# MMintLab/gelslim_depth

Measured on AMD Instinct MI355X. Metric: train frames/sec (320x427) at batch 32, higher is better.
Workload: dtype f32

## Files before the change

### gelslim_depth_amd/csrc/gsd_conv3x3_w2d.hip

```cpp
#include "gsd_common.h"

#include <cstdio>
#include <cstdlib>
#include <type_traits>

__device__ const float gsd_pad_w2d[2] = {0.f, __builtin_nanf("")};

typedef float f32x4v __attribute__((ext_vector_type(4), aligned(4)));
typedef float f32x2v __attribute__((ext_vector_type(2)));

struct W2DParams {
  SrcD src0, src1;
  DstD dst0, dst1;
  const float* wt;
  float* partials;
  const float* bw_raw;
  const float* bw_scale;
  const float* bw_shift;
  const float* bw_mean;
  const float* bw_invstd;
  int Cin, Cout, Mpad, nchunks, mblocks;
  int N, H, W;
  int TH, TW, TWq, tiles_y, tiles_x, WR, WC, WCp, PS, NPV;
  int NP, NI;
  int mgrp, pgrp, ptiles;
  int nslab;
  float* slabs;
};

namespace {
constexpr int W2D_BM = 64;
constexpr int W2D_WTILE = 96 * W2D_BM;
constexpr int NWP = 2;
}

template <class GetY>
__device__ __forceinline__ void w2d_epilogue(const W2DParams& P, const float* sBw, const int n, const int h0, const int w0, const int tr2,
                                             const int tq, const int vmask, const int m0, const int mh, const int ph, const int j,
                                             const int l16, const int pt, GetY get_y) {
  constexpr int BM = 64;
  int off0_0 = 0, off0_1 = 0, off1_0 = 0, off1_1 = 0, sm0_0 = 0, sm0_1 = 0, sm1_0 = 0, sm1_1 = 0;
#pragma unroll
  for (int a = 0; a < 2; ++a) {
    const int h = h0 + 2 * tr2 + a, w = w0 + 4 * tq;
    const int vm = (vmask >> (4 * a)) & 15;
    int hd = h - P.dst0.oh, wd = w - P.dst0.ow;
    if ((unsigned)hd < (unsigned)P.dst0.H) {
      (a == 0 ? off0_0 : off0_1) = hd * P.dst0.ws + wd;
#pragma unroll
      for (int i = 0; i < 4; ++i)
        if ((vm >> i & 1) && (unsigned)(wd + i) < (unsigned)P.dst0.W) (a == 0 ? sm0_0 : sm0_1) |= 1 << i;
    }
    hd = h - P.dst1.oh;
    wd = w - P.dst1.ow;
    if ((unsigned)hd < (unsigned)P.dst1.H) {
      (a == 0 ? off1_0 : off1_1) = hd * P.dst1.ws + wd;
#pragma unroll
      for (int i = 0; i < 4; ++i)
        if ((vm >> i & 1) && (unsigned)(wd + i) < (unsigned)P.dst1.W) (a == 0 ? sm1_0 : sm1_1) |= 1 << i;
    }
  }
  auto OFF0 = [&](int a) { return a == 0 ? off0_0 : off0_1; };
  auto OFF1 = [&](int a) { return a == 0 ? off1_0 : off1_1; };
  auto SM0 = [&](int a) { return a == 0 ? sm0_0 : sm0_1; };
  auto SM1 = [&](int a) { return a == 0 ? sm1_0 : sm1_1; };
  const long long lane0 = (long long)(j * 4) * P.dst0.cs, lane1 = (long long)(j * 4) * P.dst1.cs;
  float* const d0 = P.dst0.p + (long long)n * P.dst0.ns;
  float* const d1 = P.dst1.p + (long long)n * P.dst1.ns;
  float* const prow = P.partials != nullptr ? P.partials + (size_t)(pt * NWP + ph) * (2 * P.Mpad) : nullptr;

  if (P.bw_raw == nullptr) {
#pragma unroll
    for (int m = 0; m < 2; ++m) {
#pragma unroll
      for (int reg = 0; reg < 4; ++reg) {
        const int cu = m0 + mh * 32 + m * 16 + reg, co = cu + j * 4;
        const bool first = co < P.dst0.C;
        const int cd = first ? co : co - P.dst0.C;
        const bool co_ok = co < P.Cout && (first || cd < P.dst1.C);
        float* const plane = first ? d0 + (long long)cu * P.dst0.cs + lane0 : d1 + (long long)(cu - P.dst0.C) * P.dst1.cs + lane1;
        float y[2][4];
        get_y(m, reg, y);
        float s1 = 0.f, s2 = 0.f;
#pragma unroll
        for (int a = 0; a < 2; ++a) {
          const int sm = co_ok ? (first ? SM0(a) : SM1(a)) : 0;
          float* const px = plane + (first ? OFF0(a) : OFF1(a));
#pragma unroll
          for (int i = 0; i < 4; ++i) {
            if (sm >> i & 1) {
              s1 += y[a][i];
              s2 = fmaf(y[a][i], y[a][i], s2);
            }
          }
          if (sm == 15) {
            *reinterpret_cast<f32x4v*>(px) = f32x4{y[a][0], y[a][1], y[a][2], y[a][3]};
          } else {
#pragma unroll
            for (int i = 0; i < 4; ++i)
              if (sm >> i & 1) px[i] = y[a][i];
          }
        }
        if (prow != nullptr) {
          s1 = reduce16_to_lane15(s1);
          s2 = reduce16_to_lane15(s2);
          if (l16 == 15 && co < P.Mpad) {
            prow[co] = s1;
            prow[P.Mpad + co] = s2;
          }
        }
      }
    }
  } else {
#pragma unroll
    for (int m = 0; m < 2; ++m) {
#pragma unroll
      for (int reg = 0; reg < 4; ++reg) {
        const int cu = m0 + mh * 32 + m * 16 + reg, co = cu + j * 4;
        const long long cplane = (long long)n * P.dst0.ns + (co < P.Cout ? (long long)cu * P.dst0.cs + lane0 : 0);
        float xr[2][4];
#pragma unroll
        for (int a = 0; a < 2; ++a) {
          const float* const rp = P.bw_raw + cplane + OFF0(a);
// ... 7 lines not shown
        }
        const int cl = mh * 32 + m * 16 + j * 4 + reg;
        const float bsc = sBw[cl], bsh = sBw[BM + cl], bmu = sBw[2 * BM + cl], bis = sBw[3 * BM + cl];
        float y[2][4];
        get_y(m, reg, y);
        float s1 = 0.f, s2 = 0.f;
#pragma unroll
        for (int a = 0; a < 2; ++a) {
          const int sm = co < P.Cout ? SM0(a) : 0;
          float* const px = d0 + ((long long)cu * P.dst0.cs + lane0) + OFF0(a);
#pragma unroll
          for (int i = 0; i < 4; ++i) {
            const float x = xr[a][i];
            const float dz = ((sm >> i & 1) && fmaf(x, bsc, bsh) > 0.f) ? y[a][i] : 0.f;
            y[a][i] = dz;
            s1 += dz;
            s2 = fmaf(dz, (x - bmu) * bis, s2);
          }
          if (sm == 15) {
            *reinterpret_cast<f32x4v*>(px) = f32x4{y[a][0], y[a][1], y[a][2], y[a][3]};
          } else {
#pragma unroll
            for (int i = 0; i < 4; ++i)
              if (sm >> i & 1) px[i] = y[a][i];
          }
        }
        if (prow != nullptr) {
          s1 = reduce16_to_lane15(s1);
          s2 = reduce16_to_lane15(s2);
          if (l16 == 15 && co < P.Mpad) {
            prow[co] = s1;
            prow[P.Mpad + co] = s2;
          }
        }
      }
    }
  }
}

template <bool PLAIN, int HM = 0, bool SPLIT = false>
__global__ __launch_bounds__(128 * NWP, 2) void conv3x3_w2d_kernel(const W2DParams P) {
  constexpr bool X4 = HM == 1, U4 = HM == 2, PC = HM != 0;
  constexpr int W2D_NONE = -2147483647 - 1, W2D_PAD = -2147483647;
  static_assert(!X4 || PLAIN, "aligned 16-byte halo pieces: a plain, row-pitched source");
  constexpr int BM = W2D_BM, WTILE = W2D_WTILE, NT = 128 * NWP, NW = 2 * NWP;
  extern __shared__ __attribute__((aligned(16))) float smem[];
  const int PS = P.PS;
  const int BUF = WTILE + 4 * PS;

  const int tid = threadIdx.x, lane = tid & 63;
  const int wave8 = __builtin_amdgcn_readfirstlane(tid >> 6);
  const int ph = wave8 % NWP, fh = wave8 / NWP;
  const int j = lane >> 4, l16 = lane & 15;

  const int lid = xcd_swizzle(blockIdx.x, gridDim.x);
  int mbb = lid % P.mblocks;
  const int slab = SPLIT ? (lid / P.mblocks) % P.nslab : 0;
  int pt = SPLIT ? lid / P.mblocks / P.nslab : lid / P.mblocks;
  if (!SPLIT && P.mgrp < P.mblocks) {
    const int gsz = P.pgrp * P.mblocks;
    const int g = lid / gsz;
    int r = lid - g * gsz;
    const int p0 = g * P.pgrp;
    const int pn = min(P.pgrp, P.ptiles - p0);
    const int per = pn * P.mgrp;
    const int mg = r / per;
    r -= mg * per;
    const int gn = min(P.mgrp, P.mblocks - mg * P.mgrp);
    const int pl = r / gn;
    pt = p0 + pl;
    mbb = mg * P.mgrp + (r - pl * gn);
  }
  const int c_lo = SPLIT ? (int)((long)slab * P.nchunks / P.nslab) : 0;
  const int c_hi = SPLIT ? (int)((long)(slab + 1) * P.nchunks / P.nslab) : P.nchunks;
  const int m0 = mbb * BM;
  const int tpi = P.tiles_y * P.tiles_x;
  const int n = pt / tpi;
  const int rt = pt - n * tpi;
  const int ty = rt / P.tiles_x;
  const int h0 = ty * P.TH, w0 = (rt - ty * P.tiles_x) * P.TW;

  const int q = ph * 16 + l16;
  const bool q_ok = q < (P.TH >> 1) * P.TWq && q < 16 * NWP;
  const int tr2 = q_ok ? q / P.TWq : 0;
  const int tq = q_ok ? q - tr2 * P.TWq : 0;
  const int baddr = WTILE + j * PS + (2 * tr2) * P.WCp + 4 * tq + (PC ? 4 : 0);
  int vmask = 0;
  if (q_ok) {
#pragma unroll
    for (int a = 0; a < 2; ++a)
      if (h0 + 2 * tr2 + a < P.H) {
#pragma unroll
        for (int i = 0; i < 4; ++i)
          if (w0 + 4 * tq + i < P.W) vmask |= 1 << (4 * a + i);
      }
  }

  bool p_on[2];
  int pmask = 0;
  auto seg_offsets = [&](const int seg, int (&xo)[2], const bool mark) __attribute__((always_inline)) {
    const SrcD& S = seg ? P.src1 : P.src0;
#pragma unroll
    for (int pp = 0; pp < 2; ++pp) {
      xo[pp] = W2D_NONE;
      if constexpr (PC) {
        const int u = wave8 + NW * pp;
        p_on[pp] = u < 4 * P.NI;
        const int piece = (u % P.NI) * 64 + lane;
        const int rr = piece / P.NP, pc = piece - rr * P.NP;
        if (rr < P.WR) {
          const int gh = h0 - 1 + rr, gw = w0 - 4 + 4 * pc;
          if constexpr (X4) {
            xo[pp] = ((unsigned)gh < (unsigned)S.H && gw >= 0 && gw + 4 <= S.ws) ? gh * S.ws + gw : W2D_PAD;
          } else {
            const int hs = gh - S.oh, c0 = gw - S.ow;
            xo[pp] = W2D_PAD;
            if (S.C > 0 && (unsigned)hs < (unsigned)S.H && c0 + 3 >= 0 && c0 < S.W) {
              xo[pp] = hs * S.ws + c0;
#pragma unroll
              for (int e = 0; e < 4; ++e)
                if (mark && (c0 + e < 0 || c0 + e >= S.W)) pmask |= 1 << (8 * seg + 4 * pp + e);
            }
          }
        }
        continue;
      }
      p_on[pp] = wave8 + NW * pp < P.NPV;
      const int pos = (wave8 + NW * pp) * 64 + lane;
      const int rr = pos / P.WCp, cc = pos - rr * P.WCp;
      if (rr < P.WR && cc < P.WC) {
        const int gh = h0 - 1 + rr, gw = w0 - 1 + cc;
        const int hs = gh - S.oh, ws = gw - S.ow;
        xo[pp] = ((unsigned)hs < (unsigned)S.H && (unsigned)ws < (unsigned)S.W) ? hs * S.ws + ws : W2D_PAD;
      }
    }
  };
  int xo0[2], xo1[2];
  seg_offsets(0, xo0, true);
  seg_offsets(1, xo1, true);
  const int f_sw = P.src1.C > 0 ? P.src0.C / 4 : -1;
  const bool start1 = SPLIT && f_sw >= 0 && c_lo >= f_sw;
  {
    const float pad0 = (start1 ? P.src1.relu : P.src0.relu) ? __builtin_nanf("") : 0.f;
#pragma unroll
    for (int pp = 0; pp < 2; ++pp)
      if (p_on[pp] && (start1 ? xo1[pp] : xo0[pp]) == W2D_PAD) {
#pragma unroll
        for (int b = 0; b < 2; ++b) {
          if constexpr (PC) {
            const int u = wave8 + NW * pp;
#pragma unroll
            for (int e = 0; e < 4; ++e) smem[b * BUF + WTILE + (u / P.NI) * PS + 1 + (u % P.NI) * 256 + lane * 4 + e] = pad0;
          } else {
#pragma unroll
            for (int ch = 0; ch < 4; ++ch) smem[b * BUF + WTILE + ch * PS + (wave8 + NW * pp) * 64 + lane] = pad0;
          }
        }
      }
  }
  long long d_cs = start1 ? P.src1.cs : P.src0.cs;
  const float* d_base = (start1 ? P.src1.p + (long long)n * P.src1.ns : P.src0.p + (long long)n * P.src0.ns) +
                        (long long)(c_lo - (start1 ? f_sw : 0)) * 4 * d_cs;
  long long f_xl[2];
#pragma unroll
  for (int pp = 0; pp < 2; ++pp) f_xl[pp] = start1 ? xo1[pp] : xo0[pp];
  auto begin_fill = [&](int chunk, int buf) {
    if (f_sw < 0 || start1 || (chunk != f_sw && chunk != f_sw + 1)) return;
// ... 221 lines not shown
  };
  for (int chunk = c_lo; chunk < c_hi; chunk += 2) {
    run_chunk(chunk, std::integral_constant<int, 0>{});
    if (chunk + 1 < c_hi) run_chunk(chunk + 1, std::integral_constant<int, 1>{});
  }

  {
    float* const xs = smem + (wave8 * 12) * 256 + lane * 4;
    const float* const xr = smem + ((ph + NWP * (1 - fh)) * 12) * 256 + lane * 4;
#pragma unroll
    for (int r = 0; r < 2; ++r) {
      __syncthreads();
#pragma unroll
      for (int f = 0; f < 12; ++f) *reinterpret_cast<f32x4*>(xs + f * 256) = acc[2 + r][f];
      __syncthreads();
#pragma unroll
      for (int f = 0; f < 12; ++f) acc[2 + r][f] = *reinterpret_cast<const f32x4*>(xr + f * 256);
    }
  }

  auto out_transform = [&](auto hi_c, int m, int reg, float (&y)[2][4]) __attribute__((always_inline)) {
    constexpr bool HI = decltype(hi_c)::value;
    const int lo = HI ? 2 + m : m, hi = HI ? m : 2 + m;
    const int r0 = reg & ~1;
#pragma unroll
    for (int a = 0; a < 2; ++a) {
      f32x2v R[6];
#pragma unroll
      for (int fc = 0; fc < 6; ++fc) {
        const f32x2v M0 = {acc[lo][fc][r0], acc[lo][fc][r0 + 1]}, M1 = {acc[lo][6 + fc][r0], acc[lo][6 + fc][r0 + 1]};
        const f32x2v M2 = {acc[hi][fc][r0], acc[hi][fc][r0 + 1]}, M3 = {acc[hi][6 + fc][r0], acc[hi][6 + fc][r0 + 1]};
        R[fc] = a == 0 ? M0 + M1 + M2 : M1 - M2 - M3;
      }
      const f32x2v p12 = R[1] + R[2], m12 = R[1] - R[2], p34 = R[3] + R[4], m34 = R[3] - R[4];
      const f32x2v c2 = {2.f, 2.f}, c4 = {4.f, 4.f}, c8 = {8.f, 8.f};
      const f32x2v y0 = R[0] + p12 + p34, y1 = __builtin_elementwise_fma(c2, m34, m12), y2 = __builtin_elementwise_fma(c4, p34, p12);
      const f32x2v y3 = __builtin_elementwise_fma(c8, m34, m12) + R[5];
      y[a][0] = y0[reg & 1], y[a][1] = y1[reg & 1], y[a][2] = y2[reg & 1], y[a][3] = y3[reg & 1];
    }
  };

  auto finish = [&](auto hi_c) __attribute__((always_inline)) {
    auto get_y = [&](int m, int reg, float (&y)[2][4]) __attribute__((always_inline)) { out_transform(hi_c, m, reg, y); };
    if constexpr (SPLIT) {
      float* const sl = P.slabs + ((size_t)((size_t)pt * P.nslab + slab) * P.mblocks + mbb) * (size_t)(BM * 128 * NWP);
#pragma unroll
      for (int m = 0; m < 2; ++m)
#pragma unroll
        for (int reg = 0; reg < 4; ++reg) {
          float y[2][4];
          get_y(m, reg, y);
          float* const o = sl + ((size_t)(fh * 32 + m * 16 + j * 4 + reg) * (16 * NWP) + q) * 8;
          *reinterpret_cast<f32x4*>(o) = f32x4{y[0][0], y[0][1], y[0][2], y[0][3]};
          *reinterpret_cast<f32x4*>(o + 4) = f32x4{y[1][0], y[1][1], y[1][2], y[1][3]};
        }
    } else {
      w2d_epilogue(P, sBw, n, h0, w0, tr2, tq, vmask, m0, fh, ph, j, l16, pt, get_y);
    }
  };
  if (fh == 0)
    finish(std::false_type{});
  else
    finish(std::true_type{});
}

__global__ __launch_bounds__(128 * NWP) void w2d_slab_reduce_kernel(const W2DParams P) {
  constexpr int BM = W2D_BM;
  __shared__ float sBw[4 * BM];
  const int tid = threadIdx.x, lane = tid & 63;
  const int wave8 = __builtin_amdgcn_readfirstlane(tid >> 6);
  const int ph = wave8 % NWP, mh = wave8 / NWP;
  const int j = lane >> 4, l16 = lane & 15;
  const int lid = xcd_swizzle(blockIdx.x, gridDim.x);
  const int mbb = lid % P.mblocks;
  const int pt = lid / P.mblocks;
  const int m0 = mbb * BM;
  const int tpi = P.tiles_y * P.tiles_x;
  const int n = pt / tpi;
  const int rt = pt - n * tpi;
  const int ty = rt / P.tiles_x;
  const int h0 = ty * P.TH, w0 = (rt - ty * P.tiles_x) * P.TW;
  const int q = ph * 16 + l16;
  const bool q_ok = q < (P.TH >> 1) * P.TWq && q < 16 * NWP;
  const int tr2 = q_ok ? q / P.TWq : 0;
  const int tq = q_ok ? q - tr2 * P.TWq : 0;
  int vmask = 0;
  if (q_ok) {
#pragma unroll
    for (int a = 0; a < 2; ++a)
      if (h0 + 2 * tr2 + a < P.H) {
#pragma unroll
        for (int i = 0; i < 4; ++i)
          if (w0 + 4 * tq + i < P.W) vmask |= 1 << (4 * a + i);
      }
  }
  if (P.bw_raw != nullptr) {
    for (int c = tid; c < BM; c += 128 * NWP) {
      const int co = m0 + c < P.Cout ? m0 + c : 0;
      sBw[c] = P.bw_scale[co];
      sBw[BM + c] = P.bw_shift[co];
      sBw[2 * BM + c] = P.bw_mean[co];
      sBw[3 * BM + c] = P.bw_invstd[co];
    }
    __syncthreads();
  }
  const size_t tile_elems = (size_t)(BM * 128 * NWP);
  const float* const s0 = P.slabs + ((size_t)pt * P.nslab * P.mblocks + mbb) * tile_elems;
  auto get_y = [&](int m, int reg, float (&y)[2][4]) __attribute__((always_inline)) {
    const float* o = s0 + ((size_t)(mh * 32 + m * 16 + j * 4 + reg) * (16 * NWP) + q) * 8;
    f32x4 a = *reinterpret_cast<const f32x4*>(o), b = *reinterpret_cast<const f32x4*>(o + 4);
    for (int s = 1; s < P.nslab; ++s) {
      o += (size_t)P.mblocks * tile_elems;
      a += *reinterpret_cast<const f32x4*>(o);
      b += *reinterpret_cast<const f32x4*>(o + 4);
    }
    y[0][0] = a[0], y[0][1] = a[1], y[0][2] = a[2], y[0][3] = a[3];
    y[1][0] = b[0], y[1][1] = b[1], y[1][2] = b[2], y[1][3] = b[3];
  };
  w2d_epilogue(P, sBw, n, h0, w0, tr2, tq, vmask, m0, mh, ph, j, l16, pt, get_y);
}

namespace {

struct W2DPlan {
  int TH, TW, TWq, tiles_y, tiles_x, mblocks, WR, WC, WCp, PS;
};

int w2d_read_cycles(int TWq, int LP, int PS) {
  static const int g128[2][16] = {{0, 1, 2, 3, 12, 13, 14, 15, 20, 21, 22, 23, 24, 25, 26, 27},
                                  {4, 5, 6, 7, 8, 9, 10, 11, 16, 17, 18, 19, 28, 29, 30, 31}};
  int total = 0;
  for (int ph = 0; ph < NWP; ++ph) {
    int addr[64];
    for (int lane = 0; lane < 64; ++lane) {
      const int q = ph * 16 + (lane & 15);
      addr[lane] = (lane >> 4) * PS + 2 * (q / TWq) * LP + 4 * (q % TWq);
    }
    for (int half = 0; half < 2; ++half) {
      for (int g = 0; g < 2; ++g) {
        int worst = 0;
        for (int slot = 0; slot < 16; ++slot) {
          int distinct = 0, seen[16];
          for (int i = 0; i < 16; ++i) {
            const int a = addr[g128[g][i] + 32 * half];
            if ((a / 4) % 16 != slot) continue;
            bool dup = false;
            for (int k = 0; k < distinct; ++k) dup = dup || seen[k] == a;
            if (!dup) seen[distinct++] = a;
          }
          worst = distinct > worst ? distinct : worst;
        }
        total += worst;
      }
      int worst = 0;
      for (int slot = 0; slot < 32; ++slot) {
        int distinct = 0, seen[32];
        for (int i = 0; i < 32; ++i) {
          const int a = addr[i + 32 * half] + 4;
          if ((a / 2) % 32 != slot) continue;
          bool dup = false;
          for (int k = 0; k < distinct; ++k) dup = dup || seen[k] == a;
          if (!dup) seen[distinct++] = a;
        }
        worst = distinct > worst ? distinct : worst;
      }
      total += worst;
    }
// ... 131 lines not shown

extern "C" int64_t gsd_conv3x3_w2d_mfma_count(int N, int H, int W, int Cin, int Cout) {
  W2DPlan p;
  if (N <= 0 || H <= 0 || W <= 0 || Cin <= 0 || Cout <= 0 || !plan_w2d(N, H, W, Cout, &p)) return 0;
  return (int64_t)N * p.tiles_y * p.tiles_x * p.mblocks * ceil_div(Cin, 4) * (2 * NWP * 48);
}

extern "C" double gsd_conv3x3_w2d_estimate_us(int N, int H, int W, int Cin, int Cout) {
  W2DPlan p;
  if (N <= 0 || H <= 0 || W <= 0 || Cin <= 0 || Cout <= 0 || !plan_w2d(N, H, W, Cout, &p)) return 0.0;
  const long blocks = (long)N * p.tiles_y * p.tiles_x * p.mblocks;
  return w2d_time_us(blocks, ceil_div(Cin, 4), 1, false);
}

extern "C" double gsd_conv3x3_w2d_estimate_slabs_us(int N, int H, int W, int Cin, int Cout) {
  W2DPlan p;
  if (N <= 0 || H <= 0 || W <= 0 || Cin <= 0 || Cout <= 0 || !plan_w2d(N, H, W, Cout, &p)) return 0.0;
  const long blocks = (long)N * p.tiles_y * p.tiles_x * p.mblocks;
  return w2d_time_us(blocks, ceil_div(Cin, 4), w2d_pick_slabs(blocks, ceil_div(Cin, 4), false), false);
}

extern "C" int64_t gsd_conv3x3_w2d_workspace(int N, int H, int W, int Cin, int Cout) {
  W2DPlan p;
  if (N <= 0 || H <= 0 || W <= 0 || Cin <= 0 || Cout <= 0 || Cin % 4 != 0 || !plan_w2d(N, H, W, Cout, &p)) return 0;
  const long blocks = (long)N * p.tiles_y * p.tiles_x * p.mblocks;
  const int S = std::max(w2d_pick_slabs(blocks, Cin / 4, false), w2d_pick_slabs(blocks, Cin / 4, true));
  return S > 1 ? (int64_t)blocks * S * (W2D_BM * 256) : 0;
}

extern "C" double gsd_conv3x3_w43_estimate_us(int N, int H, int W, int Cin, int Cout, int slabs);

extern "C" int gsd_conv3x3_prefers_w2d(int N, int H, int W, int Cin, int Cout, int train) {
  if (N <= 0 || H <= 0 || W <= 0 || Cin < 16 || Cin % 4 != 0 || Cout <= 0) return 0;
  const int forced = gsd_env_int("GSD_CONV_W2D", -1);
  if (forced == 0 || forced == 1) return forced;
  if (!train) return 1;
  const double a = gsd_conv3x3_w2d_estimate_slabs_us(N, H, W, Cin, Cout), b = gsd_conv3x3_w43_estimate_us(N, H, W, Cin, Cout, 1);
  return a > 0.0 && b > 0.0 && a < b ? 1 : 0;
}

static int w2d_impl(const gsd_src* src, int nsrc, const float* wt, int Cin, int Cout, const gsd_dst* dst, int ndst, float* partials,
                    const float* bw_raw, const float* bw_scale, const float* bw_shift, const float* bw_mean, const float* bw_invstd,
                    int N, int H, int W, void* stream, float* ws = nullptr, int64_t ws_elems = 0) {
  GSD_REQUIRE(src && dst && wt, GSD_ERR_BAD_ARG, "gsd_conv3x3_w2d: null argument");
  GSD_REQUIRE(nsrc >= 1 && nsrc <= 2 && ndst >= 1 && ndst <= 2, GSD_ERR_BAD_ARG, "gsd_conv3x3_w2d: nsrc/ndst must be 1 or 2");
  GSD_REQUIRE(N > 0 && H > 0 && W > 0 && Cin > 0 && Cout > 0, GSD_ERR_BAD_ARG, "gsd_conv3x3_w2d: bad sizes");
  GSD_REQUIRE(H < 32768 && W < 32768, GSD_ERR_UNSUPPORTED, "gsd_conv3x3_w2d: H, W must be < 32768");
  GSD_REQUIRE(((uintptr_t)wt & 15) == 0, GSD_ERR_BAD_ARG, "gsd_conv3x3_w2d: weight layout must be 16-byte aligned");
  GSD_REQUIRE(gsd_conv3x3_w2d_supported(Cin, src[0].C), GSD_ERR_UNSUPPORTED,
              "gsd_conv3x3_w2d: Cin=%d and the first segment's %d channels must be multiples of 4 (use gsd_conv3x3_w43)", Cin, src[0].C);
  int csum = 0;
  for (int i = 0; i < nsrc; ++i) {
    if (int e = gsd_check_src(src[i], "gsd_conv3x3_w2d src", true)) return e;
    GSD_REQUIRE(src[i].scale == nullptr || src[i].relu != 0, GSD_ERR_UNSUPPORTED,
                "gsd_conv3x3_w2d: an affine source segment must also have relu (zero padding uses a NaN sentinel)");
    GSD_REQUIRE((int64_t)src[i].H * src[i].w_stride < (1LL << 31), GSD_ERR_UNSUPPORTED, "gsd_conv3x3_w2d: plane too large");
    csum += src[i].C;
  }
  GSD_REQUIRE(csum == Cin, GSD_ERR_BAD_ARG, "gsd_conv3x3_w2d: source segments hold %d channels, Cin=%d", csum, Cin);
  csum = 0;
  for (int i = 0; i < ndst; ++i) {
    if (int e = gsd_check_dst(dst[i], "gsd_conv3x3_w2d dst", true)) return e;
    GSD_REQUIRE((int64_t)dst[i].H * dst[i].w_stride < (1LL << 31), GSD_ERR_UNSUPPORTED, "gsd_conv3x3_w2d: plane too large");
    csum += dst[i].C;
  }
  GSD_REQUIRE(csum == Cout, GSD_ERR_BAD_ARG, "gsd_conv3x3_w2d: destination segments hold %d channels, Cout=%d", csum, Cout);

  W2DPlan pl;
  GSD_REQUIRE(plan_w2d(N, H, W, Cout, &pl), GSD_ERR_UNSUPPORTED, "gsd_conv3x3_w2d: no tile shape");
  W2DParams P;
  P.src0 = to_srcd(src[0]);
  P.src1 = nsrc > 1 ? to_srcd(src[1]) : null_srcd();
  P.dst0 = to_dstd(dst[0]);
  P.dst1 = ndst > 1 ? to_dstd(dst[1]) : null_dstd();
  P.wt = wt;
  P.partials = partials;
  P.bw_raw = bw_raw; P.bw_scale = bw_scale; P.bw_shift = bw_shift; P.bw_mean = bw_mean; P.bw_invstd = bw_invstd;
  P.Cin = Cin; P.Cout = Cout;
  P.Mpad = round_up(Cout, 64);
  P.nchunks = Cin / 4;
  P.mblocks = pl.mblocks;
  P.N = N; P.H = H; P.W = W;
  P.TH = pl.TH; P.TW = pl.TW; P.TWq = pl.TWq; P.tiles_y = pl.tiles_y; P.tiles_x = pl.tiles_x;
  P.WR = pl.WR; P.WC = pl.WC; P.WCp = pl.WCp; P.PS = pl.PS;
  P.NPV = ceil_div(P.WR * P.WCp, 64);
  GSD_REQUIRE(P.NPV <= 4 * NWP, GSD_ERR_UNSUPPORTED, "gsd_conv3x3_w2d: halo window too large");
  {
    int g = (gsd_env_int("GSD_W2D_L2KB", 3072) << 10) / (P.nchunks * W2D_WTILE * 4);
    const int forced = gsd_env_int("GSD_W2D_MGROUP", -1);
    if (forced == 0) g = P.mblocks;
    if (forced > 0) g = forced;
    P.mgrp = std::min(std::max(g, 1), P.mblocks);
    P.pgrp = std::max(gsd_env_int("GSD_W2D_PGROUP", 64 / P.mgrp), 1);
    P.ptiles = N * pl.tiles_y * pl.tiles_x;
  }
  const long base = (long)N * pl.tiles_y * pl.tiles_x * P.mblocks;
  int S = ws != nullptr ? w2d_pick_slabs(base, P.nchunks, bw_raw != nullptr) : 1;
  while (S > 1 && (int64_t)base * S * (W2D_BM * 256) > ws_elems) --S;
  if (S > 1 && P.nchunks / S < 2) S = 1;
  P.nslab = S;
  P.slabs = S > 1 ? ws : nullptr;
  if (S > 1) GSD_REQUIRE(((uintptr_t)ws & 15) == 0, GSD_ERR_BAD_ARG, "gsd_conv3x3_w2d: the K-slab workspace must be 16-byte aligned");
  const long grid = base * S;
  GSD_REQUIRE(grid < 2147483647L, GSD_ERR_UNSUPPORTED, "gsd_conv3x3_w2d: grid too large");
  bool plain = true;
  for (int i = 0; i < nsrc; ++i) plain = plain && src[i].scale == nullptr && src[i].relu == 0;
  P.NP = pl.TW / 4 + 2;
  P.NI = ceil_div(P.WR * P.NP, 64);
  const bool x4 = plain && nsrc == 1 && 4 * P.NI <= 8 && gsd_env_int("GSD_W2D_X4", 1) != 0 &&
                  ((uintptr_t)src[0].ptr & 15) == 0 && src[0].w_stride % 4 == 0 && src[0].c_stride % 4 == 0 && src[0].n_stride % 4 == 0 &&
                  src[0].off_h == 0 && src[0].off_w == 0 && src[0].w_stride >= round_up(src[0].W, 4);
  bool u4 = !x4 && 4 * P.NI <= 8 && gsd_env_int("GSD_W2D_U4", 1) != 0;
  for (int i = 0; i < nsrc && u4; ++i) u4 = src[i].slack >= 4;
  if (x4 || u4) {
    P.WCp = 4 * P.NP;
    P.PS = w2d_x4_plane_stride(pl.TWq, P.WCp, P.WR);
  }
  const size_t lds = (size_t)(2 * (W2D_WTILE + 4 * P.PS) + 2 * 4 * P.nchunks + 4 * W2D_BM) * sizeof(float);
  if (gsd_env_set("GSD_W2D_TRACE"))
    fprintf(stderr, "w2d M%d K%d %dx%d N%d nsrc %d ndst %d plain %d x4 %d u4 %d | ptr&15 %d ws %d cs%%4 %d ns%%4 %d NI %d tile %dx%d slabs %d\n", Cout, Cin, H, W, N,
            nsrc, ndst, (int)plain, (int)x4, (int)u4, (int)((uintptr_t)src[0].ptr & 15), src[0].w_stride, (int)(src[0].c_stride % 4),
            (int)(src[0].n_stride % 4), P.NI, pl.TH, pl.TW, S);
  if (S > 1) {
    if (x4) return launch_w2d<true, 1, true>(P, (int)grid, lds, (hipStream_t)stream);
    if (u4) return plain ? launch_w2d<true, 2, true>(P, (int)grid, lds, (hipStream_t)stream) : launch_w2d<false, 2, true>(P, (int)grid, lds, (hipStream_t)stream);
    return plain ? launch_w2d<true, 0, true>(P, (int)grid, lds, (hipStream_t)stream) : launch_w2d<false, 0, true>(P, (int)grid, lds, (hipStream_t)stream);
  }
  if (x4) return launch_w2d<true, 1>(P, (int)grid, lds, (hipStream_t)stream);
  if (u4) return plain ? launch_w2d<true, 2>(P, (int)grid, lds, (hipStream_t)stream) : launch_w2d<false, 2>(P, (int)grid, lds, (hipStream_t)stream);
  return plain ? launch_w2d<true>(P, (int)grid, lds, (hipStream_t)stream) : launch_w2d<false>(P, (int)grid, lds, (hipStream_t)stream);
}

extern "C" int gsd_conv3x3_w2d(const gsd_src* src, int nsrc, const float* wt, int Cin, int Cout, const gsd_dst* dst, int ndst,
                               float* partials, int N, int H, int W, void* stream) {
  return w2d_impl(src, nsrc, wt, Cin, Cout, dst, ndst, partials, nullptr, nullptr, nullptr, nullptr, nullptr, N, H, W, stream);
}

extern "C" int gsd_conv3x3_w2d_dgrad_bnrelu(const gsd_src* src, const float* wt, int Cin, int Cout, const gsd_dst* dst,
                                            const float* raw, const float* scale, const float* shift, const float* mean,
                                            const float* invstd, float* partials, int N, int H, int W, void* stream) {
  GSD_REQUIRE(dst && raw && scale && shift && mean && invstd && partials, GSD_ERR_BAD_ARG,
              "gsd_conv3x3_w2d_dgrad_bnrelu: null argument");
  GSD_REQUIRE(dst->C == Cout && dst->H == H && dst->W == W && dst->off_h == 0 && dst->off_w == 0, GSD_ERR_BAD_ARG,
              "gsd_conv3x3_w2d_dgrad_bnrelu: dst must be the full (Cout,H,W) gradient buffer (raw shares its strides)");
  return w2d_impl(src, 1, wt, Cin, Cout, dst, 1, partials, raw, scale, shift, mean, invstd, N, H, W, stream);
}

extern "C" int gsd_conv3x3_w2d_ws(const gsd_src* src, int nsrc, const float* wt, int Cin, int Cout, const gsd_dst* dst, int ndst,
                                  float* partials, float* workspace, int64_t workspace_elems, int N, int H, int W, void* stream) {
  return w2d_impl(src, nsrc, wt, Cin, Cout, dst, ndst, partials, nullptr, nullptr, nullptr, nullptr, nullptr, N, H, W, stream, workspace,
                  workspace_elems);
}

extern "C" int gsd_conv3x3_w2d_dgrad_bnrelu_ws(const gsd_src* src, const float* wt, int Cin, int Cout, const gsd_dst* dst,
                                               const float* raw, const float* scale, const float* shift, const float* mean,
                                               const float* invstd, float* partials, float* workspace, int64_t workspace_elems, int N,
                                               int H, int W, void* stream) {
  GSD_REQUIRE(dst && raw && scale && shift && mean && invstd && partials, GSD_ERR_BAD_ARG,
              "gsd_conv3x3_w2d_dgrad_bnrelu: null argument");
  GSD_REQUIRE(dst->C == Cout && dst->H == H && dst->W == W && dst->off_h == 0 && dst->off_w == 0, GSD_ERR_BAD_ARG,
              "gsd_conv3x3_w2d_dgrad_bnrelu: dst must be the full (Cout,H,W) gradient buffer (raw shares its strides)");
  return w2d_impl(src, 1, wt, Cin, Cout, dst, 1, partials, raw, scale, shift, mean, invstd, N, H, W, stream, workspace, workspace_elems);
}
```

### gelslim_depth_amd/csrc/gsd_convT.hip

```cpp
#include "gsd_common.h"

namespace {

enum : int { CT_FWD = 1, CT_DGRAD = 2 };

struct ConvTParams {
  SrcD src;
  DstD dst;
  const float* wt;
  const float* bias;
  int K, M, Mpad, nchunks, mblocks;
  int N, H, W;
  int tiles_flat;
};

template <int MODE, int WM, int WN>
__global__ __launch_bounds__(256) void convT_kernel(const ConvTParams P) {
  constexpr int MT = 4, NT = 4;
  constexpr int BM = WM * 64, BN = WN * 64;
  constexpr int KSTEPS = 4;
  constexpr int WROWS = KSTEPS * 4;
  constexpr int WS = BM + 16;
  constexpr int PS = BN + 16;
  constexpr int W4 = WROWS * BM / 4;
// ... 328 lines not shown
            const float bz = P.bias != nullptr ? P.bias[co] : 0.f;
            float* const oc = o + (long long)co * D.cs;
            *reinterpret_cast<float2*>(oc) = make_float2(acc[m][t][0] + bz, acc[m][t][1] + bz);
            *reinterpret_cast<float2*>(oc + D.ws) = make_float2(acc[m][t][2] + bz, acc[m][t][3] + bz);
          }
        }
      }
    }
  }
}

struct ConvTDgParams {
  SrcD src;
  DstD dst;
  const float* wt;
  int K, Kpad, M, nchunks, mblocks;
  int N, H, W, Wv, tiles_flat;
  const float* bw_raw;
  const float* bw_scale;
  const float* bw_shift;
  const float* bw_mean;
  const float* bw_invstd;
  float* partials;
  int Mpad;
};

template <bool BW>
__global__ __launch_bounds__(256, 2) void convT_dgrad_dma_kernel(const ConvTDgParams P) {
  constexpr int BM = 128, BN = 128, KC = 32, MT = 4, NT = 4;
  constexpr int WIMG = KC * BM, XIMG = (KC / 2) * (2 * BN), BUF = WIMG + XIMG;
  extern __shared__ __attribute__((aligned(16))) float smem[];
  const int tid = threadIdx.x, lane = tid & 63;
  const int wave = __builtin_amdgcn_readfirstlane(tid >> 6);
  const int wm = wave >> 1, wn = wave & 1;
  const int j = lane >> 4, l16 = lane & 15;

  const int lid = xcd_swizzle(blockIdx.x, gridDim.x);
  const int mb = lid % P.mblocks;
  const int pt = lid / P.mblocks;
  const int m0 = mb * BM;
  const long long q0 = (long long)pt * BN;
  const int HWv = P.H * P.Wv;
  const long long QT = (long long)P.N * HWv;

  const float* const wsrc = P.wt + (size_t)mb * P.Kpad * BM + lane * 4;
  const int pi = lane ^ ((lane >> 4) & 1);
  long long xo = 0;
  bool xok;
  {
    const long long q = q0 + 2 * pi;
    xok = q < QT;
    const int nn = xok ? (int)(q / HWv) : 0;
    const int rem = xok ? (int)(q - (long long)nn * HWv) : 0;
    const int h = rem / P.Wv, w = rem - h * P.Wv;
    xo = (long long)nn * P.src.ns + (long long)(2 * h) * P.src.ws + 2 * w;
  }
  auto fill = [&](int chunk, int buf) {
    float* Wb = smem + buf * BUF;
    float* Xb = Wb + WIMG;
    const float* wc = wsrc + (size_t)chunk * WIMG;
#pragma unroll
    for (int i = 0; i < 4; ++i) __builtin_amdgcn_global_load_lds(wc + (wave + 4 * i) * 256, Wb + (wave + 4 * i) * 256, 16, 0, 0);
#pragma unroll
    for (int i = 0; i < 4; ++i) {
      const int r = wave + 4 * i;
      const int co = chunk * 8 + (r >> 1);
      const float* g = (xok && co < P.src.C) ? P.src.p + xo + (long long)co * P.src.cs + (long long)(r & 1) * P.src.ws
                                              : &gsd_zero16_ct[0];
      __builtin_amdgcn_global_load_lds(g, Xb + r * 256, 16, 0, 0);
    }
  };

  f32x4 acc[MT][NT];
#pragma unroll
  for (int m = 0; m < MT; ++m)
#pragma unroll
    for (int t = 0; t < NT; ++t) acc[m][t] = f32x4{0.f, 0.f, 0.f, 0.f};

  const int a_off = (2 * j) * BM + wm * 64 + l16 * 4;
  const int lp = 2 * (wn * 16 + l16);
  const int b_off0 = WIMG + j * 256 + 4 * (lp ^ ((lp >> 4) & 1));
  const int b_off1 = WIMG + j * 256 + 4 * ((lp + 1) ^ (((lp + 1) >> 4) & 1));
  fill(0, 0);
  for (int chunk = 0; chunk < P.nchunks; ++chunk) {
    const int cur = chunk & 1;
    gsd_dma_barrier();
    if (chunk + 1 < P.nchunks) fill(chunk + 1, cur ^ 1);
    const float* Sb = smem + cur * BUF;
    f32x4 av[2], x0[2], x1[2];
    av[0] = *reinterpret_cast<const f32x4*>(&Sb[a_off]);
    x0[0] = *reinterpret_cast<const f32x4*>(&Sb[b_off0]);
    x1[0] = *reinterpret_cast<const f32x4*>(&Sb[b_off1]);
#pragma unroll
    for (int s = 0; s < KC / 4; ++s) {
      const int p = s >> 1, kw = s & 1, c = s & 1, pc = p & 1;
      if (s + 1 < KC / 4) {
        av[c ^ 1] = *reinterpret_cast<const f32x4*>(&Sb[a_off + ((s + 1) >> 1) * 8 * BM + ((s + 1) & 1) * BM]);
        if (kw == 1) {
          x0[pc ^ 1] = *reinterpret_cast<const f32x4*>(&Sb[b_off0 + (p + 1) * 4 * 256]);
          x1[pc ^ 1] = *reinterpret_cast<const f32x4*>(&Sb[b_off1 + (p + 1) * 4 * 256]);
        }
      }
      const float b[NT] = {x0[pc][kw], x0[pc][2 + kw], x1[pc][kw], x1[pc][2 + kw]};
#pragma unroll
      for (int m = 0; m < MT; ++m)
#pragma unroll
        for (int t = 0; t < NT; ++t) acc[m][t] = mfma16(av[c][m], b[t], acc[m][t]);
    }
  }

  typedef float f32x4u __attribute__((ext_vector_type(4), aligned(4)));
  const DstD& D = P.dst;
  const long long qa = q0 + wn * 64 + l16 * 4;
  if constexpr (BW) {
    __syncthreads();
    float* sBw = smem;
    if (tid < BM) {
      const int c = m0 + tid < D.C ? m0 + tid : 0;
      sBw[tid] = P.bw_scale[c];
      sBw[BM + tid] = P.bw_shift[c];
      sBw[2 * BM + tid] = P.bw_mean[c];
      sBw[3 * BM + tid] = P.bw_invstd[c];
    }
    __syncthreads();
    long long off[NT];
    bool ok[NT];
#pragma unroll
    for (int t = 0; t < NT; ++t) {
      const long long q = qa + t;
      ok[t] = q < QT;
      const int nn = ok[t] ? (int)(q / HWv) : 0;
      const int r = ok[t] ? (int)(q - (long long)nn * HWv) : 0;
      const int h = r / P.Wv, w = r - h * P.Wv;
      ok[t] = ok[t] && w < P.W;
      off[t] = (long long)nn * D.ns + (long long)h * D.ws + w;
    }
    const bool row4 = ok[0] && ok[3] && off[3] == off[0] + 3;
    float* const prow = P.partials + (size_t)(pt * 2 + wn) * (2 * P.Mpad);
#pragma unroll
    for (int m = 0; m < MT; ++m)
#pragma unroll
      for (int reg = 0; reg < 4; ++reg) {
        const int cl = wm * 64 + m * 16 + j * 4 + reg, ci = m0 + cl;
        const bool c_ok = ci < D.C;
        const long long cp = (long long)(c_ok ? ci : 0) * D.cs;
        const float bsc = sBw[cl], bsh = sBw[BM + cl], bmu = sBw[2 * BM + cl], bis = sBw[3 * BM + cl];
        float x[NT], dz[NT];
        if (row4) {
          const f32x4 tv = *reinterpret_cast<const f32x4u*>(P.bw_raw + cp + off[0]);
          x[0] = tv[0], x[1] = tv[1], x[2] = tv[2], x[3] = tv[3];
        } else {
#pragma unroll
          for (int t = 0; t < NT; ++t) x[t] = ok[t] ? P.bw_raw[cp + off[t]] : 0.f;
        }
        float s1 = 0.f, s2 = 0.f;
#pragma unroll
        for (int t = 0; t < NT; ++t) {
          dz[t] = (c_ok && ok[t] && fmaf(x[t], bsc, bsh) > 0.f) ? acc[m][t][reg] : 0.f;
          s1 += dz[t];
          s2 = fmaf(dz[t], (x[t] - bmu) * bis, s2);
        }
        if (c_ok) {
          if (row4) {
            *reinterpret_cast<f32x4u*>(D.p + cp + off[0]) = f32x4{dz[0], dz[1], dz[2], dz[3]};
          } else {
#pragma unroll
            for (int t = 0; t < NT; ++t)
              if (ok[t]) D.p[cp + off[t]] = dz[t];
          }
        }
        s1 = reduce16_to_lane15(s1);
        s2 = reduce16_to_lane15(s2);
        if (l16 == 15 && ci < P.Mpad) {
          prow[ci] = s1;
          prow[P.Mpad + ci] = s2;
        }
      }
    return;
  }
  if (qa < QT) {
    const int na = (int)(qa / HWv);
    const int ra = (int)(qa - (long long)na * HWv);
    const int ha = ra / P.Wv, wa = ra - ha * P.Wv;
    if (wa + 3 < P.W) {
      float* const o = D.p + (long long)na * D.ns + (long long)ha * D.ws + wa;
#pragma unroll
      for (int m = 0; m < MT; ++m)
#pragma unroll
        for (int reg = 0; reg < 4; ++reg) {
          const int ci = m0 + wm * 64 + m * 16 + j * 4 + reg;
          if (ci < D.C)
            *reinterpret_cast<f32x4u*>(o + (long long)ci * D.cs) = f32x4{acc[m][0][reg], acc[m][1][reg], acc[m][2][reg], acc[m][3][reg]};
        }
    } else {
#pragma unroll
      for (int t = 0; t < NT; ++t) {
        const long long q = qa + t;
        if (q >= QT) continue;
        const int nn = (int)(q / HWv);
        const int r = (int)(q - (long long)nn * HWv);
        const int h = r / P.Wv, w = r - h * P.Wv;
        if (w >= P.W) continue;
        float* const o = D.p + (long long)nn * D.ns + (long long)h * D.ws + w;
#pragma unroll
        for (int m = 0; m < MT; ++m)
#pragma unroll
          for (int reg = 0; reg < 4; ++reg) {
            const int ci = m0 + wm * 64 + m * 16 + j * 4 + reg;
            if (ci < D.C) o[(long long)ci * D.cs] = acc[m][t][reg];
          }
      }
    }
  }
}

template <int MODE, int WM, int WN>
int launch(const ConvTParams& P, int grid, size_t lds, hipStream_t st, const char* what) {
  hipLaunchKernelGGL((convT_kernel<MODE, WM, WN>), dim3(grid), dim3(256), lds, st, P);
  GSD_LAUNCH_CHECK(what);
  return GSD_OK;
}

template <int MODE>
int run(ConvTParams& P, hipStream_t st, const char* what) {
  const bool wide = P.M <= 64;
  const int BM = wide ? 64 : 128, BN = wide ? 256 : 128;
  P.Mpad = round_up(P.M, 64);
  P.mblocks = ceil_div(P.M, BM);
  P.tiles_flat = ceil_div(P.H * P.W, BN);
  const long grid = (long)P.N * P.tiles_flat * P.mblocks;
  GSD_REQUIRE(grid < 2147483647L, GSD_ERR_UNSUPPORTED, "%s: grid too large", what);
  const size_t lds = (size_t)(16 * (BM + 16) + 16 * (BN + 16)) * sizeof(float);
  if (wide) return launch<MODE, 1, 4>(P, (int)grid, lds, st, what);
  return launch<MODE, 2, 2>(P, (int)grid, lds, st, what);
}

}
// ... 175 lines not shown
```

Before: 368.6.

## Add interior fast-path epilogue for Winograd conv and prefetch BW inputs in convT

Adds a fast path to the Winograd 3x3 conv epilogue for tiles that lie fully inside the image and a single destination segment. It uses 32-bit offsets and unmasked float4 loads and stores, with no per-element bounds checks. The convT backward kernel now loads the raw activation and batchnorm parameters before the K loop so their latency overlaps the MFMA main loop. The cost is many extra live registers (64 floats per thread in xraw), which may reduce occupancy. It also swaps a division for a shift and requires power-of-two tile widths.

```diff
diff --git a/gelslim_depth_amd/csrc/gsd_conv3x3_w2d.hip b/gelslim_depth_amd/csrc/gsd_conv3x3_w2d.hip
--- a/gelslim_depth_amd/csrc/gsd_conv3x3_w2d.hip
+++ b/gelslim_depth_amd/csrc/gsd_conv3x3_w2d.hip
@@ -21,9 +21,10 @@
   const float* bw_invstd;
   int Cin, Cout, Mpad, nchunks, mblocks;
   int N, H, W;
-  int TH, TW, TWq, tiles_y, tiles_x, WR, WC, WCp, PS, NPV;
+  int TH, TW, TWq, TWqs, tiles_y, tiles_x, WR, WC, WCp, PS, NPV;
   int NP, NI;
   int mgrp, pgrp, ptiles;
+  int interior;
   int nslab;
   float* slabs;
 };
@@ -39,6 +40,76 @@
                                              const int tq, const int vmask, const int m0, const int mh, const int ph, const int j,
                                              const int l16, const int pt, GetY get_y) {
   constexpr int BM = 64;
+  {
+    const bool lastseg = m0 >= P.dst0.C;
+    const DstD& D = lastseg ? P.dst1 : P.dst0;
+    const int hd0 = h0 - D.oh, wd0 = w0 - D.ow;
+    const bool interior = P.interior != 0 && (P.TH >> 1) * P.TWq == 16 * NWP && h0 + P.TH <= P.H && w0 + P.TW <= P.W &&
+                          m0 + BM <= P.Cout && (lastseg || m0 + BM <= P.dst0.C) && (!lastseg || m0 - P.dst0.C + BM <= P.dst1.C) &&
+                          hd0 >= 0 && hd0 + P.TH <= D.H && wd0 >= 0 && wd0 + P.TW <= D.W;
+    if (interior) {
+      const int cb = lastseg ? m0 - P.dst0.C : m0;
+      const long long sbase = (long long)n * D.ns + (long long)(cb + mh * 32) * D.cs + (long long)hd0 * D.ws + wd0;
+      const unsigned loff = (unsigned)((j * 4) * (int)D.cs + (2 * tr2) * D.ws + 4 * tq);
+      float* const prow = P.partials != nullptr ? P.partials + (size_t)(pt * NWP + ph) * (2 * P.Mpad) : nullptr;
+      const bool bw = P.bw_raw != nullptr;
+#pragma unroll
+      for (int m = 0; m < 2; ++m) {
+#pragma unroll
+        for (int reg = 0; reg < 4; ++reg) {
+          const int co = m0 + mh * 32 + m * 16 + reg + j * 4;
+          const long long cbase = sbase + (long long)(m * 16 + reg) * D.cs;
+          float* const px = D.p + cbase;
+          f32x4 xr[2] = {f32x4{0.f, 0.f, 0.f, 0.f}, f32x4{0.f, 0.f, 0.f, 0.f}};
+          float bsc = 0.f, bsh = 0.f, bmu = 0.f, bis = 0.f;
+          if (bw) {
+            const float* const rp = P.bw_raw + cbase;
+#pragma unroll
+            for (int a = 0; a < 2; ++a) xr[a] = *reinterpret_cast<const f32x4v*>(rp + (loff + (unsigned)(a * D.ws)));
+            const int cl = mh * 32 + m * 16 + j * 4 + reg;
+            bsc = sBw[cl], bsh = sBw[BM + cl], bmu = sBw[2 * BM + cl], bis = sBw[3 * BM + cl];
+          }
+          float y[2][4], t[2][4];
+          get_y(m, reg, y);
+          if (bw) {
+#pragma unroll
+            for (int a = 0; a < 2; ++a)
+#pragma unroll
+              for (int i = 0; i < 4; ++i) {
+                const float x = xr[a][i];
+                y[a][i] = fmaf(x, bsc, bsh) > 0.f ? y[a][i] : 0.f;
+                t[a][i] = (x - bmu) * bis;
+              }
+          } else {
+#pragma unroll
+            for (int a = 0; a < 2; ++a)
+#pragma unroll
+              for (int i = 0; i < 4; ++i) t[a][i] = y[a][i];
+          }
+          float s1 = 0.f, s2 = 0.f;
+#pragma unroll
+          for (int a = 0; a < 2; ++a) {
+#pragma unroll
+            for (int i = 0; i < 4; ++i) {
+              s1 += y[a][i];
+              s2 = fmaf(y[a][i], t[a][i], s2);
+            }
+            *reinterpret_cast<f32x4v*>(px + (loff + (unsigned)(a * D.ws))) = f32x4{y[a][0], y[a][1], y[a][2], y[a][3]};
+          }
+          if (prow != nullptr) {
+            s1 = reduce16_to_lane15(s1);
+            s2 = reduce16_to_lane15(s2);
+            if (l16 == 15) {
+              prow[co] = s1;
+              prow[P.Mpad + co] = s2;
+            }
+          }
+          if (reg & 1) __builtin_amdgcn_sched_barrier(0);
+        }
+      }
+      return;
+    }
+  }
   int off0_0 = 0, off0_1 = 0, off1_0 = 0, off1_1 = 0, sm0_0 = 0, sm0_1 = 0, sm1_0 = 0, sm1_1 = 0;
 #pragma unroll
   for (int a = 0; a < 2; ++a) {
@@ -212,7 +283,7 @@
 
   const int q = ph * 16 + l16;
   const bool q_ok = q < (P.TH >> 1) * P.TWq && q < 16 * NWP;
-  const int tr2 = q_ok ? q / P.TWq : 0;
+  const int tr2 = q_ok ? q >> P.TWqs : 0;
   const int tq = q_ok ? q - tr2 * P.TWq : 0;
   const int baddr = WTILE + j * PS + (2 * tr2) * P.WCp + 4 * tq + (PC ? 4 : 0);
   int vmask = 0;
@@ -600,7 +671,7 @@
   const int h0 = ty * P.TH, w0 = (rt - ty * P.tiles_x) * P.TW;
   const int q = ph * 16 + l16;
   const bool q_ok = q < (P.TH >> 1) * P.TWq && q < 16 * NWP;
-  const int tr2 = q_ok ? q / P.TWq : 0;
+  const int tr2 = q_ok ? q >> P.TWqs : 0;
   const int tq = q_ok ? q - tr2 * P.TWq : 0;
   int vmask = 0;
   if (q_ok) {
@@ -898,7 +969,12 @@
   P.mblocks = pl.mblocks;
   P.N = N; P.H = H; P.W = W;
   P.TH = pl.TH; P.TW = pl.TW; P.TWq = pl.TWq; P.tiles_y = pl.tiles_y; P.tiles_x = pl.tiles_x;
+  P.TWqs = __builtin_ctz(pl.TWq);
+  GSD_REQUIRE((1 << P.TWqs) == pl.TWq, GSD_ERR_UNSUPPORTED, "gsd_conv3x3_w2d: tile rows of %d Winograd tiles", pl.TWq);
   P.WR = pl.WR; P.WC = pl.WC; P.WCp = pl.WCp; P.PS = pl.PS;
+  P.interior = gsd_env_int("GSD_W2D_INTERIOR", 1) != 0 ? 1 : 0;
+  for (int i = 0; i < ndst; ++i)
+    if (dst[i].c_stride < 0 || 16 * (int64_t)dst[i].c_stride + (int64_t)dst[i].H * dst[i].w_stride >= (1LL << 31)) P.interior = 0;
   P.NPV = ceil_div(P.WR * P.WCp, 64);
   GSD_REQUIRE(P.NPV <= 4 * NWP, GSD_ERR_UNSUPPORTED, "gsd_conv3x3_w2d: halo window too large");
   {
diff --git a/gelslim_depth_amd/csrc/gsd_convT.hip b/gelslim_depth_amd/csrc/gsd_convT.hip
--- a/gelslim_depth_amd/csrc/gsd_convT.hip
+++ b/gelslim_depth_amd/csrc/gsd_convT.hip
@@ -434,6 +434,49 @@
   const int b_off0 = WIMG + j * 256 + 4 * (lp ^ ((lp >> 4) & 1));
   const int b_off1 = WIMG + j * 256 + 4 * ((lp + 1) ^ (((lp + 1) >> 4) & 1));
   fill(0, 0);
+
+  typedef float f32x4u __attribute__((ext_vector_type(4), aligned(4)));
+  const DstD& D = P.dst;
+  const long long qa = q0 + wn * 64 + l16 * 4;
+  long long off[NT];
+  bool ok[NT];
+  bool row4 = false;
+  float xraw[MT][4][NT], cf[4];
+  if constexpr (BW) {
+#pragma unroll
+    for (int t = 0; t < NT; ++t) {
+      const long long q = qa + t;
+      ok[t] = q < QT;
+      const int nn = ok[t] ? (int)(q / HWv) : 0;
+      const int r = ok[t] ? (int)(q - (long long)nn * HWv) : 0;
+      const int h = r / P.Wv, w = r - h * P.Wv;
+      ok[t] = ok[t] && w < P.W;
+      off[t] = (long long)nn * D.ns + (long long)h * D.ws + w;
+    }
+    row4 = ok[0] && ok[3] && off[3] == off[0] + 3;
+#pragma unroll
+    for (int m = 0; m < MT; ++m)
+#pragma unroll
+      for (int reg = 0; reg < 4; ++reg) {
+        const int ci = m0 + wm * 64 + m * 16 + j * 4 + reg;
+        const long long cp = (long long)(ci < D.C ? ci : 0) * D.cs;
+        if (row4) {
+          const f32x4 tv = *reinterpret_cast<const f32x4u*>(P.bw_raw + cp + off[0]);
+          xraw[m][reg][0] = tv[0], xraw[m][reg][1] = tv[1], xraw[m][reg][2] = tv[2], xraw[m][reg][3] = tv[3];
+        } else {
+#pragma unroll
+          for (int t = 0; t < NT; ++t) xraw[m][reg][t] = ok[t] ? P.bw_raw[cp + off[t]] : 0.f;
+        }
+      }
+    if (tid < BM) {
+      const int c = m0 + tid < D.C ? m0 + tid : 0;
+      cf[0] = P.bw_scale[c];
+      cf[1] = P.bw_shift[c];
+      cf[2] = P.bw_mean[c];
+      cf[3] = P.bw_invstd[c];
+    }
+  }
+
   for (int chunk = 0; chunk < P.nchunks; ++chunk) {
     const int cur = chunk & 1;
     gsd_dma_barrier();
@@ -461,33 +504,16 @@
     }
   }
 
-  typedef float f32x4u __attribute__((ext_vector_type(4), aligned(4)));
-  const DstD& D = P.dst;
-  const long long qa = q0 + wn * 64 + l16 * 4;
   if constexpr (BW) {
     __syncthreads();
     float* sBw = smem;
     if (tid < BM) {
-      const int c = m0 + tid < D.C ? m0 + tid : 0;
-      sBw[tid] = P.bw_scale[c];
-      sBw[BM + tid] = P.bw_shift[c];
-      sBw[2 * BM + tid] = P.bw_mean[c];
-      sBw[3 * BM + tid] = P.bw_invstd[c];
+      sBw[tid] = cf[0];
+      sBw[BM + tid] = cf[1];
+      sBw[2 * BM + tid] = cf[2];
+      sBw[3 * BM + tid] = cf[3];
     }
     __syncthreads();
-    long long off[NT];
-    bool ok[NT];
-#pragma unroll
-    for (int t = 0; t < NT; ++t) {
-      const long long q = qa + t;
-      ok[t] = q < QT;
-      const int nn = ok[t] ? (int)(q / HWv) : 0;
-      const int r = ok[t] ? (int)(q - (long long)nn * HWv) : 0;
-      const int h = r / P.Wv, w = r - h * P.Wv;
-      ok[t] = ok[t] && w < P.W;
-      off[t] = (long long)nn * D.ns + (long long)h * D.ws + w;
-    }
-    const bool row4 = ok[0] && ok[3] && off[3] == off[0] + 3;
     float* const prow = P.partials + (size_t)(pt * 2 + wn) * (2 * P.Mpad);
 #pragma unroll
     for (int m = 0; m < MT; ++m)
@@ -498,13 +524,8 @@
         const long long cp = (long long)(c_ok ? ci : 0) * D.cs;
         const float bsc = sBw[cl], bsh = sBw[BM + cl], bmu = sBw[2 * BM + cl], bis = sBw[3 * BM + cl];
         float x[NT], dz[NT];
-        if (row4) {
-          const f32x4 tv = *reinterpret_cast<const f32x4u*>(P.bw_raw + cp + off[0]);
-          x[0] = tv[0], x[1] = tv[1], x[2] = tv[2], x[3] = tv[3];
-        } else {
-#pragma unroll
-          for (int t = 0; t < NT; ++t) x[t] = ok[t] ? P.bw_raw[cp + off[t]] : 0.f;
-        }
+#pragma unroll
+        for (int t = 0; t < NT; ++t) x[t] = xraw[m][reg][t];
         float s1 = 0.f, s2 = 0.f;
 #pragma unroll
         for (int t = 0; t < NT; ++t) {
```

New measurement: 370.9, median of 6. No clear change (+0.6%).
